# AsyncFlow-Sim/AsyncFlow

Hardware: AMD Instinct MI355X
Metric: simulated request-events/sec (2-server LB scenario, 10k replicas/GPU) (higher is better)
Workload: dtype f64

## Files before the change

asyncflow_amd/csrc/af_flow.hpp:

```cpp
#pragma once

#include <stdint.h>

#include "af_core.hpp"

namespace aff {

using af::AF_INF;
using af::d2u;
using af::u2d;

enum : uint32_t {
    FLAG_FLOW_FALLBACK = 1u << 8,
    FLOW_WHY_TIE = 1u << 9,
    FLOW_WHY_LIST = 1u << 10,
    FLOW_WHY_RING = 1u << 11,
    FLOW_WHY_RAM = 1u << 12,
    FLOW_WHY_GEN_TIE = 1u << 15,
    FLOW_WHY_MASK = FLOW_WHY_TIE | FLOW_WHY_LIST | FLOW_WHY_RING | FLOW_WHY_RAM | FLOW_WHY_GEN_TIE,
};
constexpr uint32_t kMaxServers = 16;
constexpr uint32_t kSrvSlots = 16;
enum : uint32_t { LBW_ARRIVALS = 24u, LBW_SEG_OFF = LBW_ARRIVALS + kSrvSlots, LBW_SEG_LEN = LBW_SEG_OFF + kSrvSlots,
                  LBW_PROG = LBW_SEG_LEN + kSrvSlots, LBW_SLOTS = LBW_PROG + kSrvSlots, LBW_U32 = LBW_SLOTS + kSrvSlots };
// ... 74 lines not shown
    uint32_t max_pre, max_cpu, max_post;
    double ram_scale, ram_unit;
    uint32_t off_edge, off_srv, off_ep, off_row, off_emark, off_smark, off_lb;
    uint32_t blob_bytes;
    const unsigned char* blob;
    FlowLayout L;
    const double* tick_t;
    uint32_t n_ticks;
    uint32_t n_scen;
    const uint64_t* seeds;
    uint32_t n_ovr;
    const uint32_t* ovr_param;
    const uint32_t* ovr_index;
    const double* ovr_values;
    uint32_t ovr_stride;
    const double* arrivals;
    uint32_t n_draw;
    const uint32_t* pre_flags;
    double* clock;
    uint32_t clock_cap;
    uint32_t* samples;
    uint32_t tick_cap;
    uint32_t* counts;
    uint32_t* online_hist;
    uint32_t* online_rps;
    uint32_t online_hist_bins, online_rps_buckets;
    double online_hist_scale;
    uint32_t* n_fallback;
    const uint32_t* scen_map;
    unsigned long long* prof;
};
enum : uint32_t { PROF_SETUP, PROF_GEN, PROF_SELECT, PROF_SERIES_RECV, PROF_STATION, PROF_SERVERS, PROF_SERVER_SERIES, PROF_DRAW, PROF_SEND_SERIES,
                  PROF_APPEND, PROF_COMPLETE, PROF_FLUSH, PROF_PAR_SETUP, PROF_PAR_WALK, PROF_PAR_RANK, PROF_PAR_FINAL,
                  PROF_N_PAR_ROUNDS , PROF_N_PAR_ITERS, PROF_N_PAR_LANES, PROF_N_WALKED_ROUNDS, PROF_PAR_STANDING, PROF_PAR_COMMIT_WALK, kProfSections = 22u };

enum : uint32_t { FEAT_MARKS = 1u, FEAT_ONLINE = 2u, FEAT_HBM_RING = 4u, FEAT_FAR = 64u, FEAT_ALL = 7u | FEAT_FAR, FEAT_TIEBREAK = 8u,
                  FEAT_BIGLIST = 16u, FEAT_LC = 32u, FEAT_PROF = 128u, FEAT_GENSRV = 256u, FEAT_CHAIN = 512u };
constexpr uint32_t kMaxLevels = 5u;
constexpr uint32_t kAnyLevel = 0xFFu;
template <class W, uint32_t IPL = 1u, uint32_t FEAT = FEAT_ALL>
struct Flow {
    static constexpr bool kMarks = (FEAT & FEAT_MARKS) != 0u, kOnline = (FEAT & FEAT_ONLINE) != 0u,
                          kHbmRing = (FEAT & FEAT_HBM_RING) != 0u, kTieBreak = (FEAT & FEAT_TIEBREAK) != 0u,
                          kBig = (FEAT & FEAT_BIGLIST) != 0u, kLC = (FEAT & FEAT_LC) != 0u, kFar = (FEAT & FEAT_FAR) != 0u,
                          kProf = (FEAT & FEAT_PROF) != 0u, kGen = (FEAT & FEAT_GENSRV) != 0u, kChain = (FEAT & FEAT_CHAIN) != 0u;
    static_assert(!(kChain && kLC) || kFar, "server levels behind a least-connections LB: list entries carry their in-edge (FEAT_FAR)");
    unsigned long long prof_t, prof_acc[kProfSections];
    AF_CORE void prof(uint32_t section) {
        if (kProf) {
            const unsigned long long t = W::clock();
#pragma unroll
            for (uint32_t k = 0u; k < kProfSections; ++k)
                if (k == section) prof_acc[k] += t - prof_t;
            prof_t = t;
        }
    }
    const FlowArgs& A;
    AF_PLAN_AS uint64_t* blob;
    AF_PLAN_AS uint64_t* M;
    uint32_t lane;
    uint64_t seed;

    uint32_t cursor;
    uint32_t nl0, nl1, nl2, nl3;
    double h0, h1, h2, h3;
    AF_CORE uint32_t n_list_get(uint32_t s) const { return s == 0u ? nl0 : s == 1u ? nl1 : s == 2u ? nl2 : nl3; }
    AF_CORE void n_list_set(uint32_t s, uint32_t v) {
// ... 323 lines not shown
    }
    AF_CORE bool send_finish(uint32_t e, double now, uint32_t row_now, bool have_row, double transit, double& key, bool& counted) {
        counted = false;
        const double spike = (kMarks && A.n_edge_marks != 0u) ? spike_at(e, now) : 0.0;
        key = now + (transit + spike);
        if (transit + spike < 0.0) why |= FLOW_WHY_TIE;
        if (!kFar) {
            if (samples != nullptr) add_span(e, have_row ? row_now : tick_index(now, true), tick_index(key, true), 1);
        } else if (samples != nullptr) {
            const uint32_t ib = tick_index(key, true);
            if (ib != row_now) {
                add_point(e, row_now, 1);
                const uint32_t R = A.L.ring_rows, N = A.n_ticks < A.tick_cap ? A.n_ticks : A.tick_cap;
                if ((kHbmRing && R == 0u) || ib >= N || ib - tick_base < R) add_point(e, ib, -1);
                else counted = true;
            }
        }
        return true;
    }

    AF_CORE void append(uint32_t s, bool have, double key, double t0, uint32_t aux, double sent) {
        const uint64_t m = W::ballot(have);
        const uint32_t n = n_list_get(s);
        const uint32_t pos = n + W::mbcnt(m);
        if (have) {
            list_key(s)[pos] = key;
            list_t0(s)[pos] = t0;
            if (kTieBreak) list_ts(s)[pos] = sent;
            if (s == 2u || (kFar && s == 3u)) list_aux(s)[pos] = (uint16_t)aux;
        }
        n_list_set(s, n + popc64(m));
    }

    AF_CORE uint32_t select(uint32_t s, double H_in, uint32_t room, double& okey, double& ot0, uint32_t& oaux, uint32_t hs, uint32_t level = kAnyLevel) {
        if (kBig) return select_big(s, H_in, room, okey, ot0, oaux, hs, level);
        return select_regs<IPL>(s, H_in, room, okey, ot0, oaux, hs, level);
    }
    template <uint32_t IPLx>
    AF_CORE uint32_t select_regs(uint32_t s, double H_in, uint32_t room, double& okey, double& ot0, uint32_t& oaux, uint32_t hs, uint32_t level) {
        W::sync();
        const double lo = H_get(hs);
        const double hi_t = H_in < A.total_time ? H_in : A.total_time, hi = (kFar && t_lim < hi_t) ? t_lim : hi_t;
        const uint32_t n = n_list_get(s);
        okey = AF_INF;
        ot0 = 0.0;
        oaux = 0u;
        if (!(hi > lo)) return 0u;
        if (n == 0u) {
            H_set(hs, hi);
            return 0u;
        }
        AF_PLAN_AS double* K = list_key(s);
        AF_PLAN_AS double* T0 = list_t0(s);
        AF_PLAN_AS double* TS = list_ts(s);
        AF_PLAN_AS uint16_t* AX = list_aux(s);
        double sc = 64.0 * W::rcp(hi - lo);
        if (!(sc < 1e300)) sc = 1e300;
        hist()[lane] = 0u;
        W::sync();
        double k[IPLx], t[IPLx], sent[IPLx];
        uint32_t a[IPLx], b[IPLx], slot[IPLx];
        bool valid[IPLx], elig[IPLx];
#pragma unroll
        for (uint32_t q = 0u; q < IPLx; ++q) {
            valid[q] = elig[q] = false;
            k[q] = t[q] = sent[q] = 0.0;
            a[q] = b[q] = slot[q] = 0u;
            {
                const uint32_t i = q * 64u + lane;
                valid[q] = i < n;
                k[q] = K[i];
                t[q] = T0[i];
                if (kTieBreak) sent[q] = TS[i];
                a[q] = (s == 2u || (kFar && s == 3u)) ? AX[i] : 0u;
                elig[q] = valid[q] && k[q] < hi && (!kChain || level == kAnyLevel || level_of(a[q] & (kSrvSlots - 1u)) == level);
                double x = (k[q] - lo) * sc;
                x = x < 63.0 ? x : 63.0;
                b[q] = x > 0.0 ? (uint32_t)x : 0u;
                if (elig[q]) slot[q] = W::lds_add(hist() + b[q], 1u);
            }
        }
        W::sync();
        uint32_t E;
        const uint32_t cnt = hist()[lane];
        const uint32_t base = excl_scan(cnt, E);
        uint32_t bb[IPLx], bc[IPLx];
#pragma unroll
        for (uint32_t q = 0u; q < IPLx; ++q) {
            bb[q] = W::shfl32(base, b[q]);
            bc[q] = W::shfl32(cnt, b[q]);
        }
#pragma unroll
        for (uint32_t q = 0u; q < IPLx; ++q)
            if (elig[q]) {
                sorted()[bb[q] + slot[q]] = k[q];
                if (kTieBreak) sorted_ts()[bb[q] + slot[q]] = sent[q];
            }
        W::sync();
        uint32_t rank[IPLx];
#pragma unroll
        for (uint32_t q = 0u; q < IPLx; ++q) {
            rank[q] = 0u;
            if (elig[q]) {
                const uint32_t p0 = bb[q], p1 = p0 + bc[q], me = p0 + slot[q];
                uint32_t r = p0;
                if (!kTieBreak) {
                    uint32_t c = p0;
#if defined(AF_SELECT_BUCKET_AHEAD)
                    constexpr uint32_t kAhead = AF_SELECT_BUCKET_AHEAD;
#else
                    constexpr uint32_t kAhead = 4u;
#endif
                    double kq[kAhead > 0u ? kAhead : 1u];
#pragma unroll
                    for (uint32_t u = 0u; u < kAhead; ++u) kq[u] = sorted()[p0 + u];
#pragma unroll
                    for (uint32_t u = 0u; u < kAhead; ++u) {
                        const bool in = u < bc[q];
                        r += in && kq[u] < k[q] ? 1u : 0u;
                        c += in && kq[u] <= k[q] ? 1u : 0u;
                    }
#pragma nounroll
                    for (uint32_t p = p0 + kAhead; p < p1; ++p) {
                        const double kk = sorted()[p];
                        r += kk < k[q] ? 1u : 0u;
                        c += kk <= k[q] ? 1u : 0u;
                    }
                    why |= c != r + 1u ? FLOW_WHY_TIE : 0u;
                    (void)me;
                } else
#pragma nounroll
                for (uint32_t p = p0; p < p1; ++p) {
                    const double kk = sorted()[p];
                    r += kk < k[q] ? 1u : 0u;
                    if (kk == k[q] && p != me) {
                        if (kTieBreak) {
                            const double other = sorted_ts()[p];
                            r += other < sent[q] ? 1u : 0u;
                            if (other == sent[q]) why |= FLOW_WHY_TIE;
                        } else {
                            why |= FLOW_WHY_TIE;
                        }
                    }
                }
                rank[q] = r;
            }
        }
        uint32_t n_sel = E < room ? E : room;
        n_sel = n_sel < 64u ? n_sel : 64u;
        double h_left = 0.0;
        if (n_sel < E) {
#pragma unroll
            for (uint32_t q = 0u; q < IPLx; ++q) {
                const uint64_t mb = W::ballot(elig[q] && rank[q] == n_sel);
                if (mb != 0ull) h_left = bcast_f64(k[q], (uint32_t)__builtin_ctzll(mb));
            }
        }
        uint32_t kept = 0u;
#pragma unroll
        for (uint32_t q = 0u; q < IPLx; ++q) {
            {
                const bool sel = elig[q] && rank[q] < n_sel;
                const bool keep = valid[q] && !sel;
                const uint64_t m = W::ballot(keep);
                const uint32_t pos = kept + W::mbcnt(m);
                const bool has_aux = s == 2u || (kFar && s == 3u);
                if (valid[q]) {
                    AF_PLAN_AS double* dk = sel ? out_key() + rank[q] : K + pos;
                    AF_PLAN_AS double* dt = sel ? out_t0() + rank[q] : T0 + pos;
                    *dk = k[q];
                    *dt = t[q];
                    if (kTieBreak && keep) TS[pos] = sent[q];
                    if (has_aux) {
                        if (sel) out_aux()[rank[q]] = a[q];
                        else AX[pos] = (uint16_t)a[q];
                    }
                }
                kept += popc64(m);
// ... 1710 lines not shown
```

asyncflow_amd/csrc/engine.hip:

```cpp
#include <hip/hip_runtime.h>
#include <dlfcn.h>

#include <algorithm>
#include <chrono>
#include <cmath>
#include <cstdio>
#include <cstring>
#include <functional>
#include <string>
#include <vector>

#include "../../include/asyncflow_hip.h"
#include "af_core.hpp"
#include "af_flow_host.hpp"
#include "af_plan_pack.hpp"
#include "af_pregen.hpp"
#include "af_summary.hpp"
#include "af_pooled.hpp"
#include "af_series_windows.hpp"
#include "af_series_quantiles.hpp"
#include "af_series_excursions.hpp"
#include "af_series_histogram.hpp"
#include "af_series_combined.hpp"
#include "af_series_joint.hpp"
// ... 236 lines not shown
    }
    static __device__ __forceinline__ uint32_t global_load(const uint32_t* p) {
        return __hip_atomic_load(p, __ATOMIC_RELAXED, __HIP_MEMORY_SCOPE_AGENT);
    }
    static __device__ __forceinline__ void global_fence() { __builtin_amdgcn_fence(__ATOMIC_SEQ_CST, "agent"); }
    static __device__ __forceinline__ void signal_done(uint32_t* flag, uint32_t* count) {
        __builtin_amdgcn_fence(__ATOMIC_RELEASE, "agent");
        __builtin_amdgcn_wave_barrier();
        if (threadIdx.x == 0u) {
            __hip_atomic_store(flag, 1u, __ATOMIC_RELEASE, __HIP_MEMORY_SCOPE_AGENT);
            (void)__hip_atomic_fetch_add(count, 1u, __ATOMIC_RELEASE, __HIP_MEMORY_SCOPE_SYSTEM);
        }
    }
    static __device__ __forceinline__ double rcp(double x) { return __builtin_amdgcn_rcp(x); }
    static __device__ __forceinline__ double fract(double x) { return __builtin_amdgcn_fract(x); }
    static __device__ __forceinline__ uint32_t bcast32(uint32_t v, uint32_t src) { return (uint32_t)__builtin_amdgcn_readlane((int)v, (int)src); }
    static __device__ __forceinline__ uint64_t bcast64(uint64_t v, uint32_t src) {
        const uint32_t lo = bcast32((uint32_t)v, src), hi = bcast32((uint32_t)(v >> 32), src);
        return ((uint64_t)hi << 32) | lo;
    }
    template <int CTRL, int ROW_MASK>
    static __device__ __forceinline__ uint32_t dpp(uint32_t v) {
        return (uint32_t)__builtin_amdgcn_update_dpp(0, (int)v, CTRL, ROW_MASK, 0xF, true);
    }
    static __device__ __forceinline__ uint32_t scan_incl_u32(uint32_t v) {
        v += dpp<0x111, 0xF>(v);
        v += dpp<0x112, 0xF>(v);
        v += dpp<0x114, 0xF>(v);
        v += dpp<0x118, 0xF>(v);
        v += dpp<0x142, 0xA>(v);
        v += dpp<0x143, 0xC>(v);
        return v;
    }
    static __device__ __forceinline__ uint32_t mbcnt(uint64_t m) {
        return __builtin_amdgcn_mbcnt_hi((uint32_t)(m >> 32), __builtin_amdgcn_mbcnt_lo((uint32_t)m, 0u));
    }
    static __device__ __forceinline__ unsigned long long clock() { return __builtin_amdgcn_s_memtime(); }
};

constexpr uint32_t kDoneWords = 16u;
static __device__ __forceinline__ void signal_scenario_done(const uint32_t* counter_block, uint32_t sc) {
    if (counter_block == nullptr) return;
    const uint64_t* sig = reinterpret_cast<const uint64_t*>(counter_block + kDoneWords);
    uint32_t* flags = reinterpret_cast<uint32_t*>(sig[0]);
    if (flags != nullptr) WaveHip::signal_done(flags + sc, reinterpret_cast<uint32_t*>(sig[1]));
}

#ifndef AF_FLOW_WPE
#define AF_FLOW_WPE 4
#endif
#endif
#ifndef AF_JIT
template <uint32_t IPL, uint32_t FEAT>
__global__ void __launch_bounds__(64) __attribute__((amdgpu_waves_per_eu((FEAT & aff::FEAT_GENSRV) ? 3 : AF_FLOW_WPE))) af_flow_kernel(const aff::FlowArgs a) {
    extern __shared__ __attribute__((aligned(16))) unsigned char smem[];
    if (blockIdx.x >= a.n_scen) return;
    const uint32_t sc = a.scen_map ? a.scen_map[blockIdx.x] : blockIdx.x;
    aff::Flow<WaveHip, IPL, FEAT> f(a);
    f.run((LDS_AS uint64_t*)smem, sc);
    signal_scenario_done(a.n_fallback, sc);
    if (threadIdx.x == 0u && a.n_fallback) {
        const uint32_t flags = a.counts[(size_t)sc * af::CNT_SLOTS + af::CNT_FLAGS];
        if (flags & aff::FLAG_FLOW_FALLBACK) {
            atomicAdd(a.n_fallback, 1u);
            if (flags & aff::FLOW_WHY_TIE) atomicAdd(a.n_fallback + 1, 1u);
            if (flags & aff::FLOW_WHY_LIST) atomicAdd(a.n_fallback + 2, 1u);
// ... 462 lines not shown
    KArgs args{};
    unsigned char* d_blob = nullptr;
    unsigned char* d_state = nullptr;
    size_t state_cap = 0;
    void* d_sweep = nullptr;
    size_t sweep_cap = 0;
    double* d_draws = nullptr;
    size_t draws_cap = 0;
    uint32_t* d_pre_flags = nullptr;
    size_t pre_flags_cap = 0;
    uint64_t* d_tie = nullptr;
    size_t tie_cap = 0;
    uint32_t* d_n_shared = nullptr;
    uint32_t* d_map = nullptr;
    size_t map_cap = 0;
    uint32_t* d_order = nullptr;
    size_t order_cap = 0;
    const af_summary_t* fused_sum = nullptr;
    const af_outputs_t* fused_out = nullptr;
    hipStream_t stream2 = nullptr;
    hipEvent_t ev_s0 = nullptr, ev_s1 = nullptr;
    bool fused_done = false;
    uint32_t* d_done_flags = nullptr;
    size_t done_flags_cap = 0;
    uint32_t* h_done_count = nullptr;
    uint32_t* d_done_count = nullptr;
    uint32_t* d_retry = nullptr;
    size_t retry_cap = 0;
    unsigned char* d_pool = nullptr;
    size_t pool_cap = 0;
    bool pool_poisoned = false;
    uint32_t pool_word = 0;
    int wait_value_ok = -1;
    uint64_t done_ptrs[2] = {0, 0};
    bool shared_instants_likely = false;
    hipModule_t jit_module = nullptr;
    hipFunction_t jit_lean = nullptr, jit_order3 = nullptr, jit_order2 = nullptr;
    std::string jit_spec;
    hipModule_t flow_jit_module = nullptr;
    hipFunction_t flow_jit_fn = nullptr;
    std::string flow_jit_spec;
    hipEvent_t ev3 = nullptr, ev4 = nullptr;
    size_t draw_memory_bytes = 0;
    uint32_t request_capacity = 0, fifo_capacity = 0, force_global = 0, lanes_per_wave = 0;
    uint32_t n_lb_edges = 0;
    std::vector<uint32_t> row_of_step;
    af_stats_t stats{};
    bool flow_ok = false, flow_general_servers = false, flow_chain = false;
    uint32_t flow_levels = 1u;
    uint32_t flow_lb_pos = 0u;
    std::string flow_reason;
    uint32_t flow_mode = 0, flow_list_entries = 0, flow_ring_rows = 0;
    aff::FlowArgs fargs{};
    aff::TickTable tick;
    double* d_tick = nullptr;
    double* d_arr = nullptr;
    size_t arr_cap = 0;
    uint32_t* d_arr_flags = nullptr;
    size_t arr_flags_cap = 0;
    uint32_t* d_fb = nullptr;
    uint32_t* d_slot = nullptr;
    size_t slot_cap = 0;
    unsigned long long* d_prof = nullptr;
    size_t prof_cap = 0;
    uint32_t has_lb = 0, cores_max = 1, ram_slots_max = 1;
    std::vector<double> edge_mean, edge_sigma, edge_spike;
// ... 465 lines not shown
    for (uint8_t d : e->edge_dist)
        if (d != dist_all) dist_all = 255u;
    if ((dist_all == AF_DIST_EXPONENTIAL && !std::getenv("AF_FLOW_DIST_CONST_EXP")) || std::getenv("AF_FLOW_NO_DIST_CONST")) dist_all = 255u;
    uint32_t wpe = 4u;
    if (const char* env = std::getenv("AF_FLOW_JIT_WPE")) {
        const int v = std::atoi(env);
        if (v >= 1 && v <= 8) wpe = (uint32_t)v;
    } else {
        const uint32_t lds_alloc = (P.lds + 511u) & ~511u, per_cu = lds_alloc ? (160u * 1024u) / lds_alloc : 16u;
        wpe = (per_cu + 3u) / 4u;
        wpe = wpe < 2u ? 2u : wpe > 4u ? 4u : wpe;
        if ((P.feat & (uint32_t)aff::FEAT_GENSRV) != 0u && wpe > 3u) wpe = 3u;
    }
    char buf[2048];
    std::snprintf(buf, sizeof buf,
                  "-DAF_JIT=1 -DAF_FLOW_JIT=1 -DAF_FJ_IPL=%u -DAF_FJ_FEAT=%u -DAF_FJ_TOTAL_TIME=0x%llxull -DAF_FJ_PERIOD=0x%llxull "
                  "-DAF_FJ_INV_PERIOD=0x%llxull -DAF_FJ_TICK_EPS=0x%llxull -DAF_FJ_METRICS=%u -DAF_FJ_GEN_EDGE=%u -DAF_FJ_CLIENT_EDGE=%u "
                  "-DAF_FJ_N_EDGES=%u -DAF_FJ_N_SERVERS=%u -DAF_FJ_HAS_LB=%u -DAF_FJ_N_LB=%u -DAF_FJ_N_EMARKS=%u -DAF_FJ_N_SMARKS=%u "
                  "-DAF_FJ_LC=%u -DAF_FJ_MAX_PRE=%u -DAF_FJ_MAX_CPU=%u -DAF_FJ_MAX_POST=%u -DAF_FJ_OFF_EDGE=%u -DAF_FJ_OFF_SRV=%u "
                  "-DAF_FJ_OFF_EP=%u -DAF_FJ_OFF_ROW=%u -DAF_FJ_OFF_EMARK=%u -DAF_FJ_OFF_SMARK=%u -DAF_FJ_OFF_LB=%u -DAF_FJ_BLOB_BYTES=%u "
                  "-DAF_FJ_N_TICKS=%u -DAF_FJ_HAS_CLOCK=%d -DAF_FJ_HAS_SAMPLES=%d -DAF_FJ_HAS_ONLINE=%d -DAF_FJ_HAS_OVR=%d -DAF_FJ_DIST_ALL=%u -DAF_FJ_RAM_SCALE=%.1f "
                  "-DAF_FJ_N_LEVELS=%u -DAF_FJ_LB_POS=%u -DAF_FJ_WPE=%u -DAF_FJ_LAYOUT=%u,%u,%u,%u,%u,%u,%u,%u,%u,%u,%u,%u,%u,%u,%u,%u,%u,%u,%u,%u,%u,%u,%u,%u,%u,%u,%u,%u,%u,%u",
                  P.ipl, P.feat | (std::getenv("AF_FLOW_PROF") ? (uint32_t)aff::FEAT_PROF : 0u), bits(f.total_time), bits(f.sample_period), bits(f.inv_period), bits(f.tick_eps), f.metrics_mask,
                  f.gen_out_edge, f.client_out_edge, f.n_edges, f.n_servers, f.has_lb, f.n_lb_edges, f.n_edge_marks, f.n_srv_marks,
                  f.lb_least_connections, f.max_pre, f.max_cpu, f.max_post, f.off_edge, f.off_srv, f.off_ep, f.off_row, f.off_emark,
                  f.off_smark, f.off_lb, f.blob_bytes, f.n_ticks, out->clock ? 1 : 0, out->samples ? 1 : 0,
                  (out->online_hist || out->online_rps) ? 1 : 0, has_ovr ? 1 : 0, dist_all, f.ram_scale, e->flow_levels, e->flow_lb_pos, wpe,
                  L.cap, L.ring_rows, L.win_rows, L.g_ring, L.c_ring, L.pitch, L.list_arrays, L.off_spike, L.off_list, L.off_aux, L.off_aux3,
                  L.off_out, L.off_sorted, L.off_hist, L.off_seg, L.off_fr, L.off_gr, L.off_cnt, L.off_ring, L.n_words, L.cap_of[0],
                  L.cap_of[1], L.cap_of[2], L.cap_of[3], L.off_list_of[0], L.off_list_of[1], L.off_list_of[2], L.off_list_of[3], L.off_eb, L.off_gsrv);
    std::string spec(buf);
    const bool keys = (P.feat == 0u || (P.feat & aff::FEAT_MARKS) != 0u) && (P.feat & aff::FEAT_GENSRV) == 0u;
    if (keys && !std::getenv("AF_FLOW_KEYS_HOISTED")) spec += " -DAF_FJ_KEYS_PER_CALL=1";
    return spec;
}
}

extern "C" {

int af_abi_version(void) { return AF_ABI_VERSION; }

const char* af_last_error(void) { return g_err.c_str(); }

uint32_t af_tick_count(double sample_period, double total_time) {
    if (!(sample_period > 0.0)) return 0;
    uint32_t n = 0;
    double t = 0.0 + sample_period;
    while (t < total_time) {
        n += 1;
        t = t + sample_period;
    }
    return n;
}

uint32_t af_series_count(const af_plan_t* plan) { return plan ? plan->n_edges + 3u * plan->n_servers : 0u; }

uint32_t af_series_pitch(const af_plan_t* plan) { return (af_series_count(plan) + 3u) & ~3u; }

int af_engine_create(const af_plan_t* plan, int device, const af_engine_options_t* opts, af_engine_t** out) {
    if (!out) return fail(AF_ERR_INVALID, "out is NULL");
    *out = nullptr;
    if (int rc = validate_plan(plan)) return rc;
    const bool plan_only = device == AF_DEVICE_PLAN_ONLY;
    if (!plan_only) {
        int n_dev = 0;
        if (hipGetDeviceCount(&n_dev) != hipSuccess || n_dev <= 0)
// ... 617 lines not shown

static int pick_flow_kernel(Run& r, uint32_t nc, FlowLaunch& fl) {
    af_engine_t* e = r.e;
    const FlowPlan& FP = r.FP;
    fl.lds = spread_lds_bytes(FP.lds);
    fl.jit = e->flow_jit_fn != nullptr && fl.lds <= 64u * 1024u &&
             flow_jit_spec_string(e, FP, r.out, r.sweep->n_overrides != 0u) == e->flow_jit_spec;
    if (e->flow_jit_fn != nullptr && !fl.jit) r.t.n_jit_miss += 1u;
    if (std::getenv("AF_DEBUG")) std::fprintf(stderr, "[af] flow jit spec: %s\n", flow_jit_spec_string(e, FP, r.out, r.sweep->n_overrides != 0u).c_str());
    if (std::getenv("AF_DEBUG"))
        std::fprintf(stderr, "[af] flow launch: %u scenarios, %u list entries%s, %u ring rows, %u B LDS per wave, af_flow_kernel<%u, %#x>%s%s\n", nc,
                     FP.FL.cap, FP.big ? " (long-list instantiation)" : "", FP.FL.ring_rows, FP.lds, FP.ipl, FP.feat,
                     FP.lean ? (FP.far ? ", lean instantiation with far edges" : ", lean instantiation") : "", fl.jit ? ", plan-specialised" : "");
    fl.fn = fl.jit ? nullptr : flow_kernel_for(FP.ipl, FP.feat);
    if (!fl.jit && fl.fn == nullptr) return fail(AF_ERR_INVALID, "no stage-parallel instantiation for this launch");
    if (!fl.jit && fl.lds > 48u * 1024u) HIP_TRY(hipFuncSetAttribute(fl.fn, hipFuncAttributeMaxDynamicSharedMemorySize, (int)fl.lds));
    return AF_OK;
}

static uint32_t analyzer_gate(uint32_t nc, uint32_t resident) {
    const uint32_t rem = resident ? nc % resident : 0u;
    if (resident != 0u && nc > resident && nc <= 6u * resident && rem != 0u && rem * 4u <= resident * 3u) return nc - rem;
    return 0u;
}

static int gate_for_launch(const Run& r, uint32_t nc, const FlowLaunch& fl, uint32_t& gate) {
    af_engine_t* e = r.e;
    gate = 0u;
    if (e->wait_value_ok < 0) {
        int v = 0;
        if (hipDeviceGetAttribute(&v, hipDeviceAttributeCanUseStreamWaitValue, e->device) != hipSuccess) { (void)hipGetLastError(); v = 0; }
        e->wait_value_ok = v;
    }
    int per_cu = 0;
    hipDeviceProp_t prop;
    HIP_TRY(hipGetDeviceProperties(&prop, e->device));
    if (fl.jit) HIP_TRY(hipModuleOccupancyMaxActiveBlocksPerMultiprocessor(&per_cu, e->flow_jit_fn, (int)kWave, fl.lds));
    else HIP_TRY(hipOccupancyMaxActiveBlocksPerMultiprocessor(&per_cu, fl.fn, (int)kWave, fl.lds));
    const uint32_t resident = (uint32_t)(per_cu > 0 ? per_cu : 0) * (uint32_t)prop.multiProcessorCount;
    if (e->wait_value_ok > 0) gate = analyzer_gate(nc, resident);
    if (std::getenv("AF_DEBUG")) std::fprintf(stderr, "[af] analyzer beside the last round: %u resident waves, gate at %u of %u scenarios\n", resident, gate, nc);
    return AF_OK;
}

static int arm_side_stream(af_engine_t* e, uint32_t nc) {
    if (e->stream2 == nullptr) {
        HIP_TRY(hipStreamCreateWithFlags(&e->stream2, hipStreamNonBlocking));
        HIP_TRY(hipEventCreate(&e->ev_s0));
        HIP_TRY(hipEventCreate(&e->ev_s1));
        HIP_TRY(hipHostMalloc((void**)&e->h_done_count, 64, hipHostMallocCoherent | hipHostMallocMapped));
        HIP_TRY(hipHostGetDevicePointer((void**)&e->d_done_count, e->h_done_count, 0));
    }
    if (int rc = reserve_device((void**)&e->d_done_flags, e->done_flags_cap, (size_t)nc * 4u)) return rc;
    if (int rc = reserve_device((void**)&e->d_retry, e->retry_cap, 2u * ((size_t)nc + 1u) * 4u)) return rc;
    *e->h_done_count = 0u;
    HIP_TRY(hipMemsetAsync(e->d_done_flags, 0, (size_t)nc * 4u, e->stream));
    HIP_TRY(hipMemsetAsync(e->d_retry, 0, 2u * ((size_t)nc + 1u) * 4u, e->stream));
    e->done_ptrs[0] = reinterpret_cast<uint64_t>(e->d_done_flags);
    e->done_ptrs[1] = reinterpret_cast<uint64_t>(e->d_done_count);
    HIP_TRY(hipMemcpyAsync(e->d_fb + kDoneWords, e->done_ptrs, 16u, hipMemcpyHostToDevice, e->stream));
    return AF_OK;
}

static int launch_flow(Run& r, uint32_t nc, FlowLaunch& fl) {
    af_engine_t* e = r.e;
    fl.f.n_scen = nc;
    void* kargs[] = {&fl.f};
    if (fl.jit) {
        HIP_TRY(hipModuleLaunchKernel(e->flow_jit_fn, nc, 1, 1, kWave, 1, 1, fl.lds, e->stream, kargs, nullptr));
        r.t.n_jit += 1u;
    } else {
        HIP_TRY(hipLaunchKernel(fl.fn, dim3(nc), dim3(kWave), kargs, fl.lds, e->stream));
    }
    return AF_OK;
}

static int enqueue_side_stream(af_engine_t* e, uint32_t nc, uint32_t gate) {
    auto release_side = [&]() { *e->h_done_count = 0xFFFFFFFFu; };
    hipError_t err = hipStreamWaitValue32(e->stream2, e->d_done_count, gate, hipStreamWaitValueGte, 0xFFFFFFFFu);
    if (err == hipSuccess) err = hipEventRecord(e->ev_s0, e->stream2);
    int rc = AF_OK;
    if (err == hipSuccess) rc = launch_summary_kernels(e, e->fused_out, e->fused_sum, 0u, nc, e->stream2, e->d_done_flags, e->d_retry, nullptr, 0u);
    if (err == hipSuccess && rc == AF_OK) err = hipEventRecord(e->ev_s1, e->stream2);
    if (err != hipSuccess || rc != AF_OK) {
        release_side();
        (void)hipStreamSynchronize(e->stream);
        (void)hipStreamSynchronize(e->stream2);
        if (rc != AF_OK) return rc;
        HIP_TRY(err);
    }
    return AF_OK;
}

static int dump_flow_profile(const FlowPlan& FP, uint32_t nc, const FlowLaunch& fl) {
    std::vector<unsigned long long> hp((size_t)nc * aff::kProfSections);
    HIP_TRY(hipMemcpy(hp.data(), fl.f.prof, hp.size() * 8u, hipMemcpyDeviceToHost));
    static const char* names[aff::kProfSections] = {"setup+end", "generator batch", "select", "series: delivery end (FAR)", "station logic",
                                                    "servers_solve + claim", "server series", "draws (Philox, log)", "send: spike + series",
                                                    "append + send_floor", "complete", "flush_ticks + round end",
                                                    "general servers: lanes", "general servers: walk", "general servers: rank + relax", "general servers: state at the horizon",
                                                    "COUNT rounds solved at once", "COUNT relaxation sweeps", "COUNT lanes in solved rounds", "COUNT rounds walked by event",
                                                    "general servers: standing (ranks, RAM)", "general servers: commit walk (series)"};
    double acc[aff::kProfSections] = {}, total = 0.0;
    for (uint32_t i = 0; i < nc; ++i)
        for (uint32_t k = 0; k < aff::kProfSections; ++k) acc[k] += (double)hp[(size_t)i * aff::kProfSections + k];
    for (uint32_t k = 0; k < aff::kProfSections; ++k)
        if (!names[k] || std::strncmp(names[k], "COUNT", 5) != 0) total += acc[k];
    if (FILE* fp = std::fopen(fl.prof_path, "a")) {
        std::fprintf(fp, "af_flow_kernel<%u, %#x> sections, %u waves, mean cycles per wave %.0f:\n", FP.ipl, FP.feat, nc, total / nc);
        for (uint32_t k = 0; k < aff::kProfSections; ++k)
            if (names[k]) std::fprintf(fp, "  %-28s %6.2f %%  %12.0f cycles per wave\n", names[k], 100.0 * acc[k] / total, acc[k] / nc);
        std::fclose(fp);
    }
    return AF_OK;
}

static int flow_second_chance(Run& r, const KArgs& chunk, const aff::FlowArgs& f, uint32_t lo, const std::vector<uint32_t>& retry,
                              std::vector<uint32_t>& rest, std::vector<uint32_t>& cnt_host) {
    af_engine_t* e = r.e;
    const aff::FlowLayout& FL2 = r.FP.FL2;
    if (int rc = reserve_device((void**)&e->d_map, e->map_cap, retry.size() * 4u)) return rc;
    HIP_TRY(hipMemcpyAsync(e->d_map, retry.data(), retry.size() * 4u, hipMemcpyHostToDevice, e->stream));
    aff::FlowArgs f2 = f;
    f2.L = FL2;
    f2.n_scen = (uint32_t)retry.size();
    f2.scen_map = e->d_map;
    f2.n_fallback = e->d_fb + 5;
    const uint32_t lds2 = chunk.blob_bytes + f2.L.n_words * 8u;
    if (lds2 > kLdsLimit) return fail(AF_ERR_CAPACITY, "flow kernel layout exceeds the LDS of a compute unit");
    if (chunk.online_hist || chunk.online_rps) {
        KArgs a = chunk;
        a.scen_map = e->d_map;
        hipLaunchKernelGGL(af_zero_online, dim3((uint32_t)retry.size()), dim3(256), 0, e->stream, a, (uint32_t)retry.size());
        HIP_TRY(hipGetLastError());
    }
// ... 176 lines not shown
    }
    if (on_flow) {
        const std::string spec = flow_jit_spec_string(e, FP, out, sweep->n_overrides != 0u);
        if (spec.size() + 1 > cap) return fail(AF_ERR_CAPACITY, "spec buffer too small");
        std::memcpy(buf, spec.c_str(), spec.size() + 1);
        return AF_OK;
    }
    if (e->plan_only) return fail(AF_ERR_NO_DEVICE, "planning-only engine: only sweeps of the stage-parallel kernel have a device-independent spec");
    size_t mem_free = 0, mem_total = 0;
    HIP_TRY(hipMemGetInfo(&mem_free, &mem_total));
    const uint32_t chunk = chunk_size(e, sweep->n_scenarios, (size_t)(1u + a.n_edges) * a.n_draw * sizeof(double), mem_free);
    if (chunk == 0) return fail(AF_ERR_CAPACITY, "draw_capacity too large for the device memory budget");
    uint32_t kl = 0;
    bool lds_state = false;
    choose_lanes(e, chunk, a.blob_bytes, af::layout_bytes_per_lane(a.L), kl, lds_state);
    const std::string spec = jit_spec_string(a, lds_state, klog_of(kl));
    if (spec.size() + 1 > cap) return fail(AF_ERR_CAPACITY, "spec buffer too small");
    std::memcpy(buf, spec.c_str(), spec.size() + 1);
    return AF_OK;
}

int af_engine_set_kernels(af_engine_t* e, const char* spec, const void* image, size_t size) {
    if (!e) return fail(AF_ERR_INVALID, "NULL argument");
    if (e->plan_only) return fail(AF_ERR_NO_DEVICE, "planning-only engine (AF_DEVICE_PLAN_ONLY)");
    HIP_TRY(hipSetDevice(e->device));
    const bool unload_all = !spec || !image || size == 0;
    const bool is_flow = spec && std::strstr(spec, "-DAF_FLOW_JIT=1") != nullptr;
    if (e->flow_jit_module && (unload_all || is_flow)) {
        HIP_TRY(hipStreamSynchronize(e->stream));
        (void)hipModuleUnload(e->flow_jit_module);
        e->flow_jit_module = nullptr;
        e->flow_jit_fn = nullptr;
        e->flow_jit_spec.clear();
    }
    if (is_flow && !unload_all) {
        hipModule_t mod = nullptr;
        HIP_TRY(hipModuleLoadData(&mod, image));
        hipFunction_t fn = nullptr;
        if (hipModuleGetFunction(&fn, mod, "af_flow_jit") != hipSuccess) {
            (void)hipModuleUnload(mod);
            return fail(AF_ERR_INVALID, "code object lacks af_flow_jit");
        }
        e->flow_jit_module = mod;
        e->flow_jit_fn = fn;
        e->flow_jit_spec = spec;
        return AF_OK;
    }
    if (e->jit_module) {
        HIP_TRY(hipStreamSynchronize(e->stream));
        (void)hipModuleUnload(e->jit_module);
        e->jit_module = nullptr;
        e->jit_lean = e->jit_order3 = e->jit_order2 = nullptr;
        e->jit_spec.clear();
    }
    if (!spec || !image || size == 0) return AF_OK;
    hipModule_t mod = nullptr;
    HIP_TRY(hipModuleLoadData(&mod, image));
    hipFunction_t f0 = nullptr, f1 = nullptr, f2 = nullptr;
    if (hipModuleGetFunction(&f0, mod, "af_jit_lean") != hipSuccess || hipModuleGetFunction(&f1, mod, "af_jit_order3") != hipSuccess ||
        hipModuleGetFunction(&f2, mod, "af_jit_order2") != hipSuccess) {
        (void)hipModuleUnload(mod);
        return fail(AF_ERR_INVALID, "code object lacks af_jit_lean / af_jit_order3 / af_jit_order2");
    }
    e->jit_module = mod;
    e->jit_lean = f0;
    e->jit_order3 = f1;
// ... 2563 lines not shown
```

Before: 125.7 billion.

## Rank select entries with a lane-window DPP scan before falling back to bucket sort

For single-entry-per-lane selects without tie-break or chained levels, each lane compares its quantized key against a short window of neighbouring lanes, using DPP shifts and ballots. It then confirms with a prefix-max that no farther lane is out of order. When that holds, the rank comes straight from registers and the LDS histogram, scatter and barriers are skipped; otherwise it falls back to the bucket rank. The JIT spec turns the window off for feature-enabled kernels unless an environment variable is set. Separately, the host now caches the resident-wave occupancy query per kernel and LDS size, avoiding repeated device-property calls. The window adds DPP and ballot work on every select, and a fallback costs more than before.

Result: faster. 129.6 billion, median of 6 (+3.1%).

```diff
diff --git a/asyncflow_amd/csrc/af_flow.hpp b/asyncflow_amd/csrc/af_flow.hpp
--- a/asyncflow_amd/csrc/af_flow.hpp
+++ b/asyncflow_amd/csrc/af_flow.hpp
@@ -130,7 +130,15 @@
 };
 enum : uint32_t { PROF_SETUP, PROF_GEN, PROF_SELECT, PROF_SERIES_RECV, PROF_STATION, PROF_SERVERS, PROF_SERVER_SERIES, PROF_DRAW, PROF_SEND_SERIES,
                   PROF_APPEND, PROF_COMPLETE, PROF_FLUSH, PROF_PAR_SETUP, PROF_PAR_WALK, PROF_PAR_RANK, PROF_PAR_FINAL,
-                  PROF_N_PAR_ROUNDS , PROF_N_PAR_ITERS, PROF_N_PAR_LANES, PROF_N_WALKED_ROUNDS, PROF_PAR_STANDING, PROF_PAR_COMMIT_WALK, kProfSections = 22u };
+                  PROF_N_PAR_ROUNDS , PROF_N_PAR_ITERS, PROF_N_PAR_LANES, PROF_N_WALKED_ROUNDS, PROF_PAR_STANDING, PROF_PAR_COMMIT_WALK,
+                  PROF_N_SELECT_WINDOW , PROF_N_SELECT_BUCKET, kProfSections = 24u };
+
+#ifndef AF_SELECT_WINDOW
+#define AF_SELECT_WINDOW 6
+#endif
+#if !defined(__HIPCC__)
+inline unsigned long long g_select_window_calls[2] = {0ull, 0ull};
+#endif
 
 enum : uint32_t { FEAT_MARKS = 1u, FEAT_ONLINE = 2u, FEAT_HBM_RING = 4u, FEAT_FAR = 64u, FEAT_ALL = 7u | FEAT_FAR, FEAT_TIEBREAK = 8u,
                   FEAT_BIGLIST = 16u, FEAT_LC = 32u, FEAT_PROF = 128u, FEAT_GENSRV = 256u, FEAT_CHAIN = 512u };
@@ -520,6 +528,33 @@
         n_list_set(s, n + popc64(m));
     }
 
+    AF_CORE uint32_t win_lane_below(uint32_t v) const {
+#if defined(__HIP_DEVICE_COMPILE__)
+        return W::lane_below_u32(v);
+#else
+        const uint32_t x = W::shfl32(v, (lane + 63u) & 63u);
+        return lane != 0u ? x : 0u;
+#endif
+    }
+    AF_CORE uint32_t win_prefix_max(uint32_t v) const {
+#if defined(__HIP_DEVICE_COMPILE__)
+        return W::scan_incl_max_u32(v);
+#else
+        for (uint32_t step = 1u; step < 64u; step <<= 1) {
+            const uint32_t x = W::shfl32(v, (lane + 64u - step) & 63u);
+            if (lane >= step && x > v) v = x;
+        }
+        return v;
+#endif
+    }
+    AF_CORE bool win_my_bit(uint64_t m) const {
+#if defined(__HIP_DEVICE_COMPILE__)
+        return W::my_bit(m);
+#else
+        return ((m >> lane) & 1ull) != 0ull;
+#endif
+    }
+
     AF_CORE uint32_t select(uint32_t s, double H_in, uint32_t room, double& okey, double& ot0, uint32_t& oaux, uint32_t hs, uint32_t level = kAnyLevel) {
         if (kBig) return select_big(s, H_in, room, okey, ot0, oaux, hs, level);
         return select_regs<IPL>(s, H_in, room, okey, ot0, oaux, hs, level);
@@ -544,8 +579,13 @@
         AF_PLAN_AS uint16_t* AX = list_aux(s);
         double sc = 64.0 * W::rcp(hi - lo);
         if (!(sc < 1e300)) sc = 1e300;
-        hist()[lane] = 0u;
-        W::sync();
+        constexpr uint32_t kWindow = (IPLx == 1u && !kTieBreak && !kChain) ? (uint32_t)(AF_SELECT_WINDOW) : 0u;
+        static_assert(kWindow < 32u, "AF_SELECT_WINDOW: lanes an entry looks back");
+        if (kWindow == 0u) {
+            hist()[lane] = 0u;
+            W::sync();
+        }
+        uint32_t code = 0u;
         double k[IPLx], t[IPLx], sent[IPLx];
         uint32_t a[IPLx], b[IPLx], slot[IPLx];
         bool valid[IPLx], elig[IPLx];
@@ -562,76 +602,120 @@
                 if (kTieBreak) sent[q] = TS[i];
                 a[q] = (s == 2u || (kFar && s == 3u)) ? AX[i] : 0u;
                 elig[q] = valid[q] && k[q] < hi && (!kChain || level == kAnyLevel || level_of(a[q] & (kSrvSlots - 1u)) == level);
-                double x = (k[q] - lo) * sc;
-                x = x < 63.0 ? x : 63.0;
-                b[q] = x > 0.0 ? (uint32_t)x : 0u;
-                if (elig[q]) slot[q] = W::lds_add(hist() + b[q], 1u);
-            }
-        }
-        W::sync();
-        uint32_t E;
-        const uint32_t cnt = hist()[lane];
-        const uint32_t base = excl_scan(cnt, E);
-        uint32_t bb[IPLx], bc[IPLx];
-#pragma unroll
-        for (uint32_t q = 0u; q < IPLx; ++q) {
-            bb[q] = W::shfl32(base, b[q]);
-            bc[q] = W::shfl32(cnt, b[q]);
-        }
-#pragma unroll
-        for (uint32_t q = 0u; q < IPLx; ++q)
-            if (elig[q]) {
-                sorted()[bb[q] + slot[q]] = k[q];
-                if (kTieBreak) sorted_ts()[bb[q] + slot[q]] = sent[q];
-            }
-        W::sync();
+                if (kWindow == 0u) {
+                    double x = (k[q] - lo) * sc;
+                    x = x < 63.0 ? x : 63.0;
+                    b[q] = x > 0.0 ? (uint32_t)x : 0u;
+                    if (elig[q]) slot[q] = W::lds_add(hist() + b[q], 1u);
+                } else {
+                    double y = (k[q] - lo) * (sc * 67108864.0);
+                    y = y < 4294967040.0 ? y : 4294967040.0;
+                    code = y > 1.0 ? (uint32_t)y : 1u;
+                    b[q] = code >> 26;
+                }
+            }
+        }
+        uint32_t E = 0u;
         uint32_t rank[IPLx];
-#pragma unroll
-        for (uint32_t q = 0u; q < IPLx; ++q) {
-            rank[q] = 0u;
-            if (elig[q]) {
-                const uint32_t p0 = bb[q], p1 = p0 + bc[q], me = p0 + slot[q];
-                uint32_t r = p0;
-                if (!kTieBreak) {
-                    uint32_t c = p0;
+        bool ranked = false;
+        if constexpr (kWindow != 0u) {
+            const uint32_t own = elig[0] ? code : 0xFFFFFFFFu;
+            uint32_t c[kWindow + 1u];
+            c[0] = win_lane_below(elig[0] ? code : 0u);
+#pragma unroll
+            for (uint32_t d = 1u; d <= kWindow; ++d) c[d] = win_lane_below(c[d - 1u]);
+            const uint64_t em = W::ballot(elig[0]);
+            uint32_t r = W::mbcnt(em);
+            uint64_t same = 0ull;
+#pragma unroll
+            for (uint32_t d = 1u; d <= kWindow; ++d) {
+                const bool later_in_front = c[d - 1u] > own;
+                const uint64_t m = W::ballot(later_in_front);
+                same |= W::ballot(c[d - 1u] == own);
+                r -= later_in_front ? 1u : 0u;
+                r += win_my_bit(m >> d) ? 1u : 0u;
+            }
+            const uint32_t far_max = win_prefix_max(c[kWindow]);
+            ranked = W::ballot(!(own > far_max)) == 0ull && same == 0ull;
+            rank[0] = r;
+            E = popc64(em);
+            if (kProf) {
+                if (ranked) prof_acc[PROF_N_SELECT_WINDOW] += 1ull;
+                else prof_acc[PROF_N_SELECT_BUCKET] += 1ull;
+            }
+#if !defined(__HIPCC__)
+            if (lane == 0u) g_select_window_calls[ranked ? 0 : 1] += 1ull;
+#endif
+            if (!ranked) {
+                hist()[lane] = 0u;
+                W::sync();
+                if (elig[0]) slot[0] = W::lds_add(hist() + b[0], 1u);
+            }
+        }
+        if (!ranked) {
+            W::sync();
+            const uint32_t cnt = hist()[lane];
+            const uint32_t base = excl_scan(cnt, E);
+            uint32_t bb[IPLx], bc[IPLx];
+#pragma unroll
+            for (uint32_t q = 0u; q < IPLx; ++q) {
+                bb[q] = W::shfl32(base, b[q]);
+                bc[q] = W::shfl32(cnt, b[q]);
+            }
+#pragma unroll
+            for (uint32_t q = 0u; q < IPLx; ++q)
+                if (elig[q]) {
+                    sorted()[bb[q] + slot[q]] = k[q];
+                    if (kTieBreak) sorted_ts()[bb[q] + slot[q]] = sent[q];
+                }
+            W::sync();
+#pragma unroll
+            for (uint32_t q = 0u; q < IPLx; ++q) {
+                rank[q] = 0u;
+                if (elig[q]) {
+                    const uint32_t p0 = bb[q], p1 = p0 + bc[q], me = p0 + slot[q];
+                    uint32_t r = p0;
+                    if (!kTieBreak) {
+                        uint32_t c = p0;
 #if defined(AF_SELECT_BUCKET_AHEAD)
-                    constexpr uint32_t kAhead = AF_SELECT_BUCKET_AHEAD;
+                        constexpr uint32_t kAhead = AF_SELECT_BUCKET_AHEAD;
 #else
-                    constexpr uint32_t kAhead = 4u;
+                        constexpr uint32_t kAhead = 4u;
 #endif
-                    double kq[kAhead > 0u ? kAhead : 1u];
-#pragma unroll
-                    for (uint32_t u = 0u; u < kAhead; ++u) kq[u] = sorted()[p0 + u];
-#pragma unroll
-                    for (uint32_t u = 0u; u < kAhead; ++u) {
-                        const bool in = u < bc[q];
-                        r += in && kq[u] < k[q] ? 1u : 0u;
-                        c += in && kq[u] <= k[q] ? 1u : 0u;
-                    }
+                        double kq[kAhead > 0u ? kAhead : 1u];
+#pragma unroll
+                        for (uint32_t u = 0u; u < kAhead; ++u) kq[u] = sorted()[p0 + u];
+#pragma unroll
+                        for (uint32_t u = 0u; u < kAhead; ++u) {
+                            const bool in = u < bc[q];
+                            r += in && kq[u] < k[q] ? 1u : 0u;
+                            c += in && kq[u] <= k[q] ? 1u : 0u;
+                        }
 #pragma nounroll
-                    for (uint32_t p = p0 + kAhead; p < p1; ++p) {
+                        for (uint32_t p = p0 + kAhead; p < p1; ++p) {
+                            const double kk = sorted()[p];
+                            r += kk < k[q] ? 1u : 0u;
+                            c += kk <= k[q] ? 1u : 0u;
+                        }
+                        why |= c != r + 1u ? FLOW_WHY_TIE : 0u;
+                        (void)me;
+                    } else
+#pragma nounroll
+                    for (uint32_t p = p0; p < p1; ++p) {
                         const double kk = sorted()[p];
                         r += kk < k[q] ? 1u : 0u;
-                        c += kk <= k[q] ? 1u : 0u;
-                    }
-                    why |= c != r + 1u ? FLOW_WHY_TIE : 0u;
-                    (void)me;
-                } else
-#pragma nounroll
-                for (uint32_t p = p0; p < p1; ++p) {
-                    const double kk = sorted()[p];
-                    r += kk < k[q] ? 1u : 0u;
-                    if (kk == k[q] && p != me) {
-                        if (kTieBreak) {
-                            const double other = sorted_ts()[p];
-                            r += other < sent[q] ? 1u : 0u;
-                            if (other == sent[q]) why |= FLOW_WHY_TIE;
-                        } else {
-                            why |= FLOW_WHY_TIE;
+                        if (kk == k[q] && p != me) {
+                            if (kTieBreak) {
+                                const double other = sorted_ts()[p];
+                                r += other < sent[q] ? 1u : 0u;
+                                if (other == sent[q]) why |= FLOW_WHY_TIE;
+                            } else {
+                                why |= FLOW_WHY_TIE;
+                            }
                         }
                     }
-                }
-                rank[q] = r;
+                    rank[q] = r;
+                }
             }
         }
         uint32_t n_sel = E < room ? E : room;
diff --git a/asyncflow_amd/csrc/engine.hip b/asyncflow_amd/csrc/engine.hip
--- a/asyncflow_amd/csrc/engine.hip
+++ b/asyncflow_amd/csrc/engine.hip
@@ -292,6 +292,18 @@
         v += dpp<0x143, 0xC>(v);
         return v;
     }
+    static __device__ __forceinline__ uint32_t umax(uint32_t a, uint32_t b) { return a > b ? a : b; }
+    static __device__ __forceinline__ uint32_t scan_incl_max_u32(uint32_t v) {
+        v = umax(v, dpp<0x111, 0xF>(v));
+        v = umax(v, dpp<0x112, 0xF>(v));
+        v = umax(v, dpp<0x114, 0xF>(v));
+        v = umax(v, dpp<0x118, 0xF>(v));
+        v = umax(v, dpp<0x142, 0xA>(v));
+        v = umax(v, dpp<0x143, 0xC>(v));
+        return v;
+    }
+    static __device__ __forceinline__ uint32_t lane_below_u32(uint32_t v) { return dpp<0x138, 0xF>(v); }
+    static __device__ __forceinline__ bool my_bit(uint64_t m) { return __builtin_amdgcn_inverse_ballot_w64(m); }
     static __device__ __forceinline__ uint32_t mbcnt(uint64_t m) {
         return __builtin_amdgcn_mbcnt_hi((uint32_t)(m >> 32), __builtin_amdgcn_mbcnt_lo((uint32_t)m, 0u));
     }
@@ -820,6 +832,11 @@
     bool pool_poisoned = false;
     uint32_t pool_word = 0;
     int wait_value_ok = -1;
+    struct ResidentWaves {
+        const void* fn;
+        uint32_t lds, waves;
+    };
+    std::vector<ResidentWaves> resident_waves;
     uint64_t done_ptrs[2] = {0, 0};
     bool shared_instants_likely = false;
     hipModule_t jit_module = nullptr;
@@ -1351,6 +1368,7 @@
     std::string spec(buf);
     const bool keys = (P.feat == 0u || (P.feat & aff::FEAT_MARKS) != 0u) && (P.feat & aff::FEAT_GENSRV) == 0u;
     if (keys && !std::getenv("AF_FLOW_KEYS_HOISTED")) spec += " -DAF_FJ_KEYS_PER_CALL=1";
+    if (P.feat != 0u && !std::getenv("AF_FLOW_SELECT_WINDOW_ALL")) spec += " -DAF_SELECT_WINDOW=0";
     return spec;
 }
 }
@@ -2034,12 +2052,22 @@
         if (hipDeviceGetAttribute(&v, hipDeviceAttributeCanUseStreamWaitValue, e->device) != hipSuccess) { (void)hipGetLastError(); v = 0; }
         e->wait_value_ok = v;
     }
-    int per_cu = 0;
-    hipDeviceProp_t prop;
-    HIP_TRY(hipGetDeviceProperties(&prop, e->device));
-    if (fl.jit) HIP_TRY(hipModuleOccupancyMaxActiveBlocksPerMultiprocessor(&per_cu, e->flow_jit_fn, (int)kWave, fl.lds));
-    else HIP_TRY(hipOccupancyMaxActiveBlocksPerMultiprocessor(&per_cu, fl.fn, (int)kWave, fl.lds));
-    const uint32_t resident = (uint32_t)(per_cu > 0 ? per_cu : 0) * (uint32_t)prop.multiProcessorCount;
+    const void* fn = fl.jit ? (const void*)e->flow_jit_fn : fl.fn;
+    uint32_t resident = 0u;
+    bool known = false;
+    for (const af_engine_t::ResidentWaves& rw : e->resident_waves)
+        if (rw.fn == fn && rw.lds == fl.lds) {
+            resident = rw.waves;
+            known = true;
+        }
+    if (!known) {
+        int per_cu = 0, n_cu = 0;
+        HIP_TRY(hipDeviceGetAttribute(&n_cu, hipDeviceAttributeMultiprocessorCount, e->device));
+        if (fl.jit) HIP_TRY(hipModuleOccupancyMaxActiveBlocksPerMultiprocessor(&per_cu, e->flow_jit_fn, (int)kWave, fl.lds));
+        else HIP_TRY(hipOccupancyMaxActiveBlocksPerMultiprocessor(&per_cu, fl.fn, (int)kWave, fl.lds));
+        resident = (uint32_t)(per_cu > 0 ? per_cu : 0) * (uint32_t)(n_cu > 0 ? n_cu : 0);
+        e->resident_waves.push_back({fn, fl.lds, resident});
+    }
     if (e->wait_value_ok > 0) gate = analyzer_gate(nc, resident);
     if (std::getenv("AF_DEBUG")) std::fprintf(stderr, "[af] analyzer beside the last round: %u resident waves, gate at %u of %u scenarios\n", resident, gate, nc);
     return AF_OK;
@@ -2102,7 +2130,8 @@
                                                     "append + send_floor", "complete", "flush_ticks + round end",
                                                     "general servers: lanes", "general servers: walk", "general servers: rank + relax", "general servers: state at the horizon",
                                                     "COUNT rounds solved at once", "COUNT relaxation sweeps", "COUNT lanes in solved rounds", "COUNT rounds walked by event",
-                                                    "general servers: standing (ranks, RAM)", "general servers: commit walk (series)"};
+                                                    "general servers: standing (ranks, RAM)", "general servers: commit walk (series)",
+                                                    "COUNT selects ranked by the lane window", "COUNT selects that fell back to the bucket rank"};
     double acc[aff::kProfSections] = {}, total = 0.0;
     for (uint32_t i = 0; i < nc; ++i)
         for (uint32_t k = 0; k < aff::kProfSections; ++k) acc[k] += (double)hp[(size_t)i * aff::kProfSections + k];
@@ -2345,6 +2374,7 @@
         e->flow_jit_module = nullptr;
         e->flow_jit_fn = nullptr;
         e->flow_jit_spec.clear();
+        e->resident_waves.clear();
     }
     if (is_flow && !unload_all) {
         hipModule_t mod = nullptr;
```
